# fchchen/omni-recall-rag

Measured on AMD Instinct MI355X. Metric: queries/sec at top-k=10 over N x 3072-d chunks; score delta vs C# reference in `parity`, higher is better.
Workload: dtype i8 screen + f32*f32->f64 exact re-score; 1 GPU; C3: 10000000 chunks x 3072-d fp32 on one GPU, batch=256 queries per step, top-k=10, full hybrid (cosine+keyword+recency), candidate_limit=corpus; corpus_rows=10000000

## Files before the change

### omni-recall-rag_amd/csrc/orr_api.hip

```cpp
#include <hip/hip_runtime.h>

#include <algorithm>
#include <cmath>
#include <cstdarg>
#include <cstdio>
#include <chrono>
#include <pthread.h>
#include <dlfcn.h>
#include <atomic>
#include <condition_variable>
#include <functional>
#include <cstring>
#include <limits>
#include <mutex>
#include <shared_mutex>
#include <deque>
#include <new>
#include <numeric>
#include <string>
#include <string_view>
#include <thread>
#include <unordered_map>
#include <vector>

#include "orr_escalation.h"
#include "orr_insert_plan.h"
#include "orr_kernels.h"
#include "orr_keyword_plan.h"
#include "orr_lanes.h"
#include "orr_scope_plan.h"
#include "orr_mask_plan.h"
#include "orr_group_plan.h"
#include "orr_scope_set_plan.h"
#include "orr_scope_terms_plan.h"
#include "orr_scope_near_plan.h"
#include "orr_range_bulk_plan.h"
#include "orr_cluster_handle_plan.h"
#include "orr_cluster_group_plan.h"
#include "orr_cluster_scope_plan.h"
#include "orr_cluster_diverse_plan.h"
#include "orr_cluster_per_key_plan.h"
#include "orr_token_index.h"

namespace {

thread_local std::string g_last_error = "";

int fail(int code, const char *fmt, ...)
{
    char buf[512];
    va_list ap;
    va_start(ap, fmt);
    vsnprintf(buf, sizeof(buf), fmt, ap);
    va_end(ap);
    g_last_error = buf;
    return code;
}

// ... 2630 lines not shown
    Empty,
    Exact,
    StreamMfma,
    SplitAll,
    SplitFused,
    TwoStageGemm,
    TwoStageStream,
    LargeK,
};

enum class Screen { None, I8Ranges, GemvI8, GemvBf16, Bf16Shadow, Bf16x1 };

struct PassPlan {
    PassForm form = PassForm::Exact;
    Screen screen = Screen::None;
    bool use_cos = false;
    bool use_mfma = false;
    bool q_on_device = false;
    bool dev_norms = false;
    bool prefix_i8 = false;
    bool split_queries = false;
    bool batched_score = false;
    bool rowc_inline = false;
    int32_t fused_sample_seg = 0;
    int64_t dotf_rows = 0;
    int n_ranges = 1;
    int64_t range_row[17] = {};
    int32_t count_bits = 0;
    int prefix_floor_form = 0;
    double approx_eps = 0.0;
    double eps1 = 0.0;
    bool masked = false;
    bool grouped = false;

    bool two_stage() const {
        return form == PassForm::TwoStageGemm || form == PassForm::TwoStageStream;
    }
    bool stream() const { return form == PassForm::TwoStageStream; }
    double plane_bytes_per_row(int32_t B) const { return (count_bits == 2 ? 8.0 : 16.0) * (double)((B + 31) / 32); }
    bool fused() const { return fused_sample_seg > 0; }
    int pass_mode() const { static constexpr int kMode[] = {0, 1, 1, 2, 2, 3}; return grouped ? 6 : masked ? 5 : kMode[(int)screen]; }
};

static bool has_tiny_query(const float *q, int32_t B, int32_t D)
{
    for (int32_t b = 0; b < B; ++b) {
        float mx = 0.f;
        for (int32_t k = 0; k < D; ++k) mx = std::max(mx, std::fabs(q[(size_t)b * D + k]));
        if (mx > 0.f && mx < 0x1p-48f) return true;
    }
    return false;
}

int plan_form(orr_index *idx, const BatchArgs &a, int32_t kprime, int64_t n, const std::vector<uint32_t> &qoff, PassPlan &p)
{
    const int32_t B = a.B, D = idx->dim;
    const int32_t n_seg_all = (int32_t)((n + orr::kSelSegRows - 1) / orr::kSelSegRows);
    const bool small_k = kprime <= orr::kSelWidth;
    const bool floor_fits = !a.no_fuse && n_seg_all >= 48 && std::max<int32_t>(1, a.topk) <= orr::kSelWidth;
    p = PassPlan{};
    p.use_cos = a.dim > 0 && a.dim == D;
    p.q_on_device = p.use_cos && is_device_pointer(a.q);
    const bool force_exact = a.force_exact || (p.use_cos && (idx->opt_two_stage != 1 || D % 128 != 0) && !p.q_on_device &&
                                               has_tiny_query(a.q, B, D));
    bool stream = false, stream_i8 = false;
    if (p.use_cos && !force_exact && idx->opt_two_stage == 1 && D % 64 == 0 && small_k && floor_fits && B <= orr::kMaxGemvScreenQ) {
// ... 90 lines not shown
    const uint32_t *chunks = nullptr;
    int64_t words = 0;
    std::vector<int64_t> took, n_clip, sample;
    const int64_t *d_clip = nullptr;
    const int64_t *d_sample = nullptr;
    bool floor_heads = false;
    std::vector<int32_t> qgroup;
    uint32_t cap = 0;
    const uint32_t *d_qgroup = nullptr;
    const int64_t *d_took = nullptr;
    uint32_t *h_screened = nullptr;
};

struct PassIo {
    const float *d_q = nullptr;
    double *d_dot = nullptr;
    float *d_dotf = nullptr;
    orr::KwView kw{nullptr, 0, nullptr, nullptr, nullptr};
    const double2 *d_rowc = nullptr;
    orr_candidate *d_cand = nullptr;
    bool direct_host = false;
    const MaskScope *mask = nullptr;
    GroupScopes *groups = nullptr;
};

struct PassFront {
    std::vector<uint32_t> qoff;
    uint32_t n_terms_total = 0;
    size_t rec_bytes = 0;
    bool q_download_pending = false;
    PassIo io;
};

template <class Plan>
int open_pass(orr_index *idx, const BatchArgs &a, int32_t kprime, Plan &&plan, bool pinned_records, bool out_dev, bool dev_norms,
              const float **q_host, PassPlan &p, PassFront &f)
{
    const int32_t B = a.B;
    hipStream_t s = idx->stream;
    if (q_host) *q_host = nullptr;
    f.qoff.resize((size_t)B + 1);
    memcpy(f.qoff.data(), a.query_term_off, sizeof(uint32_t) * ((size_t)B + 1));
    for (int32_t b = 0; b < B; ++b) {
        if (f.qoff[b + 1] < f.qoff[b]) return fail(ORR_EINVAL, "query_term_off is not monotone at query %d", b);
        if (f.qoff[b + 1] - f.qoff[b] > 65535) return fail(ORR_EINVAL, "query %d has more than 65535 terms", b);
    }
    f.n_terms_total = f.qoff[B] - f.qoff[0];
    if (f.n_terms_total > 0 && (!a.term_off || !a.terms_utf8)) return fail(ORR_EINVAL, "terms are referenced but term_off/terms_utf8 is NULL");

    ORR_TRY(plan(f.qoff, p));
    if (!dev_norms) p.dev_norms = false;
    idx->h_survivors.clear();

    PassIo &io = f.io;
    f.rec_bytes = sizeof(orr_candidate) * (size_t)B * ((size_t)kprime + 1);
    io.direct_host = pinned_records && !p.use_mfma && f.rec_bytes <= (256u << 10);
    if (io.direct_host) {
        ORR_TRY(idx->pin_cand.reserve(f.rec_bytes));
        io.d_cand = idx->pin_cand.as<orr_candidate>();
    } else if (out_dev && a.out_dev) {
        io.d_cand = a.out_dev;
    } else {
        ORR_TRY(idx->ws_cand.reserve(f.rec_bytes));
        io.d_cand = idx->ws_cand.as<orr_candidate>();
    }

    idx->h_norm_a.assign((size_t)B, 0.0);
    if (!p.use_cos) return ORR_OK;
    const size_t qbytes = sizeof(float) * (size_t)B * a.dim;
    if (p.dev_norms) {
        io.d_q = a.q;
        ORR_TRY(idx->ws_norm_a.reserve(sizeof(double) * (size_t)B));
        ORR_TRY(idx->pin_norm.reserve(sizeof(double) * (size_t)B));
        HIP_TRY(orr::launch_dot_exact(io.d_q, B, a.dim, nullptr, 1, true, idx->ws_norm_a.as<double>(), B, idx->stream_aux));
        HIP_TRY(hipEventRecord(idx->ev_q, idx->stream_aux));
        return ORR_OK;
    }
    ORR_TRY(idx->pin_q.reserve(qbytes));
    if (p.q_on_device) {
        io.d_q = a.q;
        HIP_TRY(hipMemcpyAsync(idx->pin_q.p, a.q, qbytes, hipMemcpyDeviceToHost, idx->stream_kw));
        HIP_TRY(hipEventRecord(idx->ev_q, idx->stream_kw));
        f.q_download_pending = true;
    } else {
// ... 173 lines not shown
        if (host_records && !a.out_dev && rec_bytes <= (256u << 10)) {
            ORR_TRY(idx->pin_cand.reserve(rec_bytes));
            io.d_cand = idx->pin_cand.as<orr_candidate>();
            io.direct_host = true;
        }
        Timed t(idx, "finish_survivors", 0.0);
        HIP_TRY(orr::launch_finish_survivors(idx->d_emb, idx->dim, io.d_q, B, idx->d_norm_b, idx->d_created, idx->d_row_ids, io.kw,
                                             idx->ws_qc.as<orr::QueryConst>(), a.now_ticks, epi.cnt, idx->ws_fcnt.as<uint32_t>() + 2 * B,
                                             kCap, epi.buf, idx->ws_fdot.as<double>(), idx->ws_sel.as<orr::SelEntry>(), kprime, n,
                                             idx->row_base, idx->ws_tsL.as<double>(), io.d_cand, idx->pin_cnt.as<uint32_t>(), s));
    } else {
        ORR_TRY(rescore_survivors(idx, a, io, epi, kCap, how, rescore_bytes, s));
        {
            Timed t(idx, "buffer_to_lists", 0.0);
            HIP_TRY(orr::launch_buffer_to_lists(epi.buf, epi.cnt, kCap, B, 0, buf_lists, idx->ws_sel.as<orr::SelEntry>(), s));
        }
        {
            Timed t(idx, "select_final", (double)B * (double)buf_lists * orr::kSelWidth * sizeof(orr::SelEntry));
            HIP_TRY(orr::launch_select_final(idx->ws_sel.as<orr::SelEntry>(), buf_lists, B, kprime, n, idx->row_base,
                                             nullptr, nullptr, 0, idx->d_norm_b, idx->d_created, idx->d_row_ids, io.kw,
                                             0, 0.0, nullptr, epi.cnt, kCap, idx->ws_tsL.as<double>(), io.d_cand, s));
        }
        {
            Timed t(idx, "records_dot_from_buffer", 0.0);
            HIP_TRY(orr::launch_records_dot_from_buffer(epi.buf, idx->ws_fdot.as<double>(), epi.cnt, kCap, B, kprime, idx->row_base,
                                                        io.d_cand, s));
        }
        if (how == Rescore::BufferExact)
            HIP_TRY(hipMemcpyAsync(idx->pin_cnt.p, epi.cnt, sizeof(uint32_t) * (size_t)B, hipMemcpyDeviceToHost, s));
    }
    return ORR_OK;
}

int screen_i8_in_ranges(orr_index *idx, const BatchArgs &a, const PassPlan &p, int64_t n, const orr::KwView &kw,
                        orr::FusedEpilogue epi, hipStream_t s)
{
    const int32_t B = a.B;
    const int64_t *range_row = p.range_row;
    if (p.n_ranges > 1) {
        hipStream_t k = idx->stream_kw;
        HIP_TRY(hipEventRecord(idx->ev_main_ready, s));
        HIP_TRY(hipStreamWaitEvent(k, idx->ev_main_ready, 0));
        for (int r = 1; r < p.n_ranges; ++r) {
            {
                Timed t(idx, "count_planes", p.plane_bytes_per_row(B) * (double)(range_row[r + 1] - range_row[r]), k);
                HIP_TRY(orr::launch_query_count_planes(kw, B, n, epi.plane_stride, idx->ws_fany.as<uint32_t>(), k, range_row[r],
                                                       range_row[r + 1], epi.count_bits == 2 ? 2 : 4));
            }
            HIP_TRY(hipEventRecord(idx->ev_range[r - 1], k));
        }
    }
    for (int r = 0; r < p.n_ranges; ++r) {
        if (r > 0) HIP_TRY(hipStreamWaitEvent(s, idx->ev_range[r - 1], 0));
        epi.tickets = idx->ws_tickets.as<uint32_t>() + 8 * r;
        const double rows_r = (double)(range_row[r + 1] - range_row[r]);
        Timed t(idx, "screen_i8_fused", rows_r * ((double)idx->dim + 32.0 + (epi.count_planes ? (epi.count_bits == 2 ? 8.0 : 16.0) * (double)((B + 31) / 32) : 0.0)) +
                                        1.0 * (double)B * idx->dim);
        HIP_TRY(orr::launch_screen_i8(idx->ws_qtiled.p, B, idx->emb_i8.p, range_row[r + 1], idx->dim, epi, s, range_row[r]));
    }
    return ORR_OK;
}

orr_index *capture_handle(orr_index *lane) { return lane->internal_lane && lane->parent ? const_cast<orr_index *>(lane->parent) : lane; }

int capture_screen(orr_index *idx, const BatchArgs &a, const PassPlan &p, int64_t n, const PassIo &io, const orr::FloorOut &floor,
                   const orr::FusedEpilogue &epi, uint32_t kCap, int32_t kth, hipStream_t s)
{
    ScreenCapture &c = capture_handle(idx)->capture;
    const size_t B = (size_t)a.B;
    c.armed.store(0, std::memory_order_relaxed);
    c.have = false;
    c.floor_key.resize(B); c.L.resize(B); c.cnt.resize(B); c.buf.resize(B * (size_t)kCap);
    HIP_TRY(hipMemcpyAsync(c.floor_key.data(), floor.floor_key, sizeof(unsigned long long) * B, hipMemcpyDeviceToHost, s));
    HIP_TRY(hipMemcpyAsync(c.L.data(), floor.L, sizeof(double) * B, hipMemcpyDeviceToHost, s));
    HIP_TRY(hipMemcpyAsync(c.cnt.data(), epi.cnt, sizeof(uint32_t) * B, hipMemcpyDeviceToHost, s));
    HIP_TRY(hipMemcpyAsync(c.buf.data(), epi.buf, sizeof(orr::SelEntry) * B * (size_t)kCap, hipMemcpyDeviceToHost, s));
    HIP_TRY(hipStreamSynchronize(s));
    orr_screen_capture &o = c.info;
    o = orr_screen_capture{};
    o.B = a.B; o.kth = kth; o.cap = kCap;
    o.screen = (int32_t)p.screen;
    o.tile_form = p.screen == Screen::I8Ranges ? orr::screen_i8_form(a.B, p.range_row[1], idx->dim, epi) : -1;
    o.scope = io.groups ? 2 : io.mask ? 1 : 0;
    o.floor_form = io.mask || p.stream() ? -1 : p.prefix_floor_form;
    o.n = n;
    o.prefix_rows = io.mask ? io.mask->sample : std::min<int64_t>(p.dotf_rows, n);
// ... 88 lines not shown
                HIP_TRY(orr::launch_screen_gemv_i8(idx->ws_q8.p, idx->ws_q8s1.as<float>(), idx->ws_q8err.as<double>(), B, idx->emb_i8.p,
                                                   idx->i8_scale.as<float>(), idx->i8_rel_err.as<float>(), idx->i8_rel_hat.as<float>(),
                                                   idx->d_norm_b, idx->d_created, a.now_ticks, pre_rows, idx->dim, pre, true, s));
            else
                HIP_TRY(orr::launch_screen_gemv_bf16(idx->ws_qsplit.p, B, idx->emb_shadow.p, pre_rows, idx->dim, pre, s));
        }
        {
            Timed t(idx, "select_floor", 0.0);
            const int32_t lists_all = (int32_t)(cap_p / orr::kSelWidth);
            const int32_t lists_p = pre_lists ? (int32_t)((pre_rows + orr::kSelWidth - 1) / orr::kSelWidth) : lists_all;
            if (!pre_lists)
                HIP_TRY(orr::launch_buffer_to_lists(pre.buf, pre.cnt, cap_p, B, 0, lists_all, idx->ws_psel.as<orr::SelEntry>(), s));
            HIP_TRY(orr::launch_select_final_sample(idx->ws_psel.as<orr::SelEntry>(), lists_all, lists_p, B, kth, d_tau, s, floor));
        }
    } else {
        if (!io.mask) {
            Timed t(idx, "select_floor", 0.0);
            HIP_TRY(orr::launch_select_final_sample(idx->ws_sel.as<orr::SelEntry>(), lists_total, p.fused_sample_seg, B, kth, d_tau, s, floor,
                                                    p.prefix_floor_form == 2 ? 1 : 0));
        }
        const bool gemm_i8 = p.screen == Screen::I8Ranges;
        if (gemm_i8) {
            epi.i8_rowf = idx->i8_rowf.as<float4>();
            epi.i8_qs1 = idx->ws_q8s1.as<float>();
        }
        HIP_TRY(orr::launch_fused_query_consts(idx->ws_qc.as<orr::QueryConst>(), idx->ws_tskey.as<unsigned long long>(), B,
                                               idx->ws_fqf.as<float4>(), s, gemm_i8 ? idx->ws_q8s1.as<float>() : nullptr,
                                               gemm_i8 ? idx->ws_q8err.as<double>() + B : nullptr,
                                               gemm_i8 ? idx->ws_fqf.as<float4>() + B : nullptr,
                                               idx->ws_fcnt.as<uint32_t>(), 3 * B, idx->ws_tickets.as<uint32_t>(), 8 * 16));
        epi.qf16 = gemm_i8 ? idx->ws_fqf.as<float4>() + B : nullptr;
    }
    epi.tau = idx->ws_tskey.as<unsigned long long>();
    if (p.screen == Screen::I8Ranges) {
        ORR_TRY(screen_i8_in_ranges(idx, a, p, n, io.kw, epi, s));
    } else if (p.screen == Screen::GemvI8) {
        Timed t(idx, "screen_gemv_i8", 1.0 * (double)n * idx->dim + 28.0 * (double)n + 2.0 * (double)B * idx->dim);
        HIP_TRY(orr::launch_screen_gemv_i8(idx->ws_q8.p, idx->ws_q8s1.as<float>(), idx->ws_q8err.as<double>(), B, idx->emb_i8.p,
                                           idx->i8_scale.as<float>(), idx->i8_rel_err.as<float>(), idx->i8_rel_hat.as<float>(),
                                           io.mask ? nullptr : idx->d_norm_b, idx->d_created, a.now_ticks, n, idx->dim, epi, false, s));
    } else if (p.screen == Screen::GemvBf16) {
        Timed t(idx, "screen_gemv_bf16", 2.0 * (double)n * idx->dim + 2.0 * (double)B * idx->dim);
        HIP_TRY(orr::launch_screen_gemv_bf16(idx->ws_qsplit.p, B, idx->emb_shadow.p, n, idx->dim, epi, s));
    } else if (p.screen == Screen::Bf16Shadow) {
        ORR_TRY(idx->ws_qtiled.reserve(orr::bf16_tiled_bytes(B, idx->dim)));
        HIP_TRY(orr::launch_bf16_tiled(io.d_q, B, idx->dim, idx->ws_qtiled.p, s));
        Timed t(idx, "screen_bf16_fused", 2.0 * (double)n * idx->dim + 2.0 * (double)B * idx->dim);
        HIP_TRY(orr::launch_screen_bf16(idx->ws_qtiled.p, B, idx->emb_shadow.p, 0, n, idx->dim, nullptr, 0, &epi, s));
    } else {
        Timed t(idx, "gemm_dot_bf16x1_fused", 4.0 * (double)n * idx->dim + 2.0 * (double)B * idx->dim);
        HIP_TRY(orr::launch_gemm_dot_bf16x3(idx->ws_qsplit.p, B, idx->d_emb, 0, n, idx->dim, nullptr, 0, &epi, 1, s));
    }
    if (io.groups) {
        if (idx->profiling == 1 && io.groups->h_screened)
            HIP_TRY(hipMemcpyAsync(io.groups->h_screened, epi.cnt, sizeof(uint32_t) * (size_t)B, hipMemcpyDeviceToHost, s));
        Timed t(idx, "mask_survivors_grouped", 16.0 * (double)B * (double)kCap);
        HIP_TRY(orr::launch_mask_survivors_grouped(io.groups->bm, io.groups->words, io.groups->n_groups, io.groups->d_clip, io.groups->d_qgroup,
                                                   epi.cnt, kCap, epi.buf, B, s));
    } else if (io.mask) {
        Timed t(idx, "mask_survivors", 16.0 * (double)B * (double)kCap);
        HIP_TRY(orr::launch_mask_survivors(io.mask->bm, io.mask->n_clip, epi.cnt, kCap, epi.buf, B, s));
    }
    if (capture_handle(idx)->capture.armed.load(std::memory_order_relaxed)) ORR_TRY(capture_screen(idx, a, p, n, io, floor, epi, kCap, kth, s));
    ORR_TRY(two_stage_tail(idx, a, kprime, n, io, epi, kCap, buf_lists, host_records, rec_bytes, Rescore::BufferExact, 0.0, s));
    if (io.groups) HIP_TRY(orr::launch_mask_trailers_grouped(io.d_cand, B, kprime, io.groups->d_took, s));
    else if (io.mask) HIP_TRY(orr::launch_mask_trailers(io.d_cand, B, kprime, io.mask->took, s));
// ... 2 lines not shown

int select_fused(orr_index *idx, const BatchArgs &a, const PassPlan &p, int32_t kprime, int64_t n, PassIo &io, bool host_records,
                 size_t rec_bytes)
{
    const int32_t B = a.B;
    hipStream_t s = idx->stream;
    uint32_t kCap = idx->survivor_cap;
    if (io.groups && io.groups->cap) kCap = io.groups->cap;
    while (kCap > 8192 && (size_t)B * kCap * 40 > ((size_t)2 << 30)) kCap >>= 1;
    idx->pass_cap = kCap;
    const int32_t fss = p.fused_sample_seg;
    const int32_t buf_lists = (int32_t)(kCap / orr::kSelWidth);
    const int32_t lists_total = fss + buf_lists;
    const int32_t finish_group = orr::finish_survivors_group(B, idx->dim);
    const int32_t lists_room = std::max<int32_t>(lists_total, finish_group ? (int32_t)(kCap / (uint32_t)finish_group) : 0);
    ORR_TRY(idx->ws_sel.reserve(sizeof(orr::SelEntry) * (size_t)B * (size_t)lists_room * orr::kSelWidth));
    ORR_TRY(idx->ws_tau.reserve(sizeof(unsigned long long) * (size_t)B));
    ORR_TRY(idx->ws_fcnt.reserve(sizeof(uint32_t) * 3 * (size_t)B));
    ORR_TRY(idx->ws_fbuf.reserve(sizeof(orr::SelEntry) * (size_t)B * kCap));
    unsigned long long *d_tau = idx->ws_tau.as<unsigned long long>();
    if (!p.stream() && !io.mask) {
        Timed t(idx, "fuse_select", (double)B * (double)p.dotf_rows * 28.0);
        orr::I8Prefix i8p;
        if (p.prefix_i8) { i8p.rowf = idx->i8_rowf.as<float4>(); i8p.qs1 = idx->ws_q8s1.as<float>(); i8p.qerr2 = idx->ws_q8err.as<double>() + B; }
        HIP_TRY(orr::launch_fuse_select(nullptr, io.d_dotf, p.dotf_rows, idx->d_norm_b, idx->d_created, io.d_rowc, io.kw,
                                        idx->ws_qc.as<orr::QueryConst>(), a.now_ticks, std::min<int64_t>(p.dotf_rows, n), B, 0, fss,
                                        nullptr, idx->ws_sel.as<orr::SelEntry>(), lists_total, s, i8p,
                                        p.prefix_floor_form));
    }
    ORR_TRY(idx->ws_fqf.reserve(sizeof(float4) * 2 * (size_t)B));
    orr::FusedEpilogue epi{};
    epi.plane_stride = (n + 63) / 64 * 64;
    if (io.kw.bitmaps && !p.stream()) {
        ORR_TRY(idx->ws_fany.reserve(sizeof(uint32_t) * orr::kCountPlanes * (size_t)((B + 31) / 32) * (size_t)epi.plane_stride));
        epi.count_bits = p.count_bits;
        Timed t(idx, "count_planes", p.plane_bytes_per_row(B) * (double)(p.range_row[1] - p.range_row[0]));
        HIP_TRY(orr::launch_query_count_planes(io.kw, B, n, epi.plane_stride, idx->ws_fany.as<uint32_t>(), s, 0, p.range_row[1],
                                               epi.count_bits == 2 ? 2 : 4));
        epi.count_planes = idx->ws_fany.as<uint32_t>();
    }
    epi.qf = idx->ws_fqf.as<float4>();
    epi.rowc = io.d_rowc; epi.qc = idx->ws_qc.as<orr::QueryConst>(); epi.kw = io.kw;
    epi.cnt = idx->ws_fcnt.as<uint32_t>(); epi.buf = idx->ws_fbuf.as<orr::SelEntry>(); epi.cap = kCap;
    if (p.screen == Screen::GemvBf16) HIP_TRY(hipMemsetAsync(idx->ws_fcnt.p, 0, sizeof(uint32_t) * 3 * (size_t)B, s));
    ORR_TRY(idx->ws_tickets.reserve(sizeof(uint32_t) * 8 * 16));
    if (p.two_stage()) return screen_two_stage(idx, a, p, kprime, n, io, epi, kCap, buf_lists, lists_total, host_records, rec_bytes);

    {
        Timed t(idx, "select_floor", 0.0);
        HIP_TRY(orr::launch_select_final_sample(idx->ws_sel.as<orr::SelEntry>(), lists_total, fss, B, kprime, d_tau, s));
    }
    HIP_TRY(orr::launch_fused_query_consts(idx->ws_qc.as<orr::QueryConst>(), d_tau, B, idx->ws_fqf.as<float4>(), s, nullptr, nullptr, nullptr,
                                           idx->ws_fcnt.as<uint32_t>(), 3 * B));
    epi.tau = d_tau;
    {
        Timed t(idx, "gemm_dot_bf16x3_fused", 4.0 * (double)(n - p.dotf_rows) * idx->dim + 4.0 * (double)B * idx->dim);
        HIP_TRY(orr::launch_gemm_dot_bf16x3(idx->ws_qsplit.p, B, idx->d_emb, p.dotf_rows, n, idx->dim, nullptr, 0, &epi, 3, s));
    }
    {
        Timed t(idx, "buffer_to_lists", 0.0);
        HIP_TRY(orr::launch_buffer_to_lists(epi.buf, epi.cnt, kCap, B, fss, lists_total, idx->ws_sel.as<orr::SelEntry>(), s));
    }
    Timed t(idx, "select_final", (double)B * (double)lists_total * orr::kSelWidth * sizeof(orr::SelEntry));
    HIP_TRY(orr::launch_select_final(idx->ws_sel.as<orr::SelEntry>(), lists_total, B, kprime, n, idx->row_base,
                                     nullptr, nullptr, 0, idx->d_norm_b, idx->d_created, idx->d_row_ids, io.kw,
                                     0, p.approx_eps, nullptr, epi.cnt, kCap, nullptr, io.d_cand, s));
    return ORR_OK;
}

int launch_selection(orr_index *idx, const BatchArgs &a, const PassPlan &p, int32_t kprime, int64_t n, PassIo &io, bool host_records,
                     size_t rec_bytes)
{
    const int32_t B = a.B;
    hipStream_t s = idx->stream;
    if (p.form == PassForm::LargeK)
        return run_large_k(idx, a, kprime, n, io.d_dot, io.kw, idx->pin_qc.as<orr::QueryConst>(), io.d_cand, s);
    const int64_t n_seg = (n + orr::kSelSegRows - 1) / orr::kSelSegRows;
    const int32_t n_seg32 = (int32_t)n_seg;
    ORR_TRY(idx->ws_sel.reserve(sizeof(orr::SelEntry) * (size_t)B * (size_t)n_seg * orr::kSelWidth));
    if (p.fused()) {
        ORR_TRY(select_fused(idx, a, p, kprime, n, io, host_records, rec_bytes));
    } else {
        const orr::QueryConst *qc = idx->ws_qc.as<orr::QueryConst>();
        unsigned long long *d_tau = nullptr;
        const int32_t sample_seg = (B >= 8 && n_seg32 >= 48) ? std::min<int32_t>(64, std::max<int32_t>(16, n_seg32 / 16)) : 0;
        if (sample_seg > 0) {
            ORR_TRY(idx->ws_tau.reserve(sizeof(unsigned long long) * (size_t)B));
// ... 80 lines not shown
    }
    g_ht.mark(4);
    collect_events(idx);
    return check_hit_list(idx, kws, nullptr);
}

int run_shard_once(orr_index *idx, const BatchArgs &a, int32_t kprime, bool host_records, const float **q_host,
                   const orr_candidate **recs_host, PassPlan &p)
{
    g_ht.start();
    ORR_TRY(bind_device(idx));
    const int64_t n = participating_rows(idx, a.candidate_limit);
    const int32_t B = a.B;
    hipStream_t s = idx->stream;
    if (recs_host) *recs_host = nullptr;

    PassFront f;
    ORR_TRY(open_pass(idx, a, kprime, [&](const std::vector<uint32_t> &qoff, PassPlan &plan) { return plan_pass(idx, a, kprime, n, qoff, plan); },
                      host_records, true, true, q_host, p, f));
    PassIo &io = f.io;

    if (p.form == PassForm::Empty) {
        const std::vector<orr_candidate> empty = empty_records(B, kprime);
        if (io.direct_host) memcpy(io.d_cand, empty.data(), f.rec_bytes);
        else HIP_TRY(hipMemcpyAsync(io.d_cand, empty.data(), f.rec_bytes, hipMemcpyHostToDevice, s));
        HIP_TRY(hipStreamSynchronize(s));
        if (f.q_download_pending || p.dev_norms) HIP_TRY(hipEventSynchronize(idx->ev_q));
        if (recs_host && io.direct_host) *recs_host = io.d_cand;
        return ORR_OK;
    }

    if (p.screen == Screen::GemvI8) ORR_TRY(launch_i8_query_image(idx, io.d_q, B, false, s));

    KwSide kws;
    ORR_TRY(launch_keyword_side(idx, a, f.qoff, kws));
    io.kw = kws.view;
    g_ht.mark(1);

    ORR_TRY(launch_numerators(idx, a, p, n, io));
    g_ht.mark(0);

    ORR_TRY(launch_consts(idx, a, p, n, f.qoff, f.q_download_pending, io));
    if (f.n_terms_total > 0) HIP_TRY(hipStreamWaitEvent(s, idx->ev_kw_done, 0));
    g_ht.mark(2);

    ORR_TRY(launch_selection(idx, a, p, kprime, n, io, host_records, f.rec_bytes));

    if (!owner_of(idx)->dead.empty())
        HIP_TRY(orr::launch_mark_dead_records(io.d_cand, B, kprime, owner_of(idx)->d_dead.as<int64_t>(),
                                              (int32_t)owner_of(idx)->dead.size(), idx->row_base, s));
    if (host_records) ORR_TRY(records_to_host(idx, f, s));
    g_ht.mark(3);
    idx->sstats.pass_mode = p.pass_mode();

    const int r = finish_pass(idx, a, p, kws, f.n_terms_total);
    if (r != ORR_OK) return r;
    if (recs_host && io.direct_host) *recs_host = io.d_cand;
    else if (recs_host && host_records) *recs_host = idx->pin_cand.as<orr_candidate>();
    return ORR_OK;
}

template <class Pass>
int retry_pass(orr_index *idx, Pass &&once)
{
    for (int attempt = 0;; ++attempt) {
        const int r = once();
        if (r != kRetryPass) return r;
        idx->sstats.passes += 1;
        if (attempt + 1 >= keyword::kMaxRuns) return hit_list_kept_overflowing(nullptr);
    }
}

int run_shard(orr_index *idx, const BatchArgs &a, int32_t kprime, bool host_records, const float **q_host,
              const orr_candidate **recs_host, PassPlan &pass)
{
    return retry_pass(idx, [&] { return run_shard_once(idx, a, kprime, host_records, q_host, recs_host, pass); });
// ... 616 lines not shown
}


struct ScopeSource {
    const ScopeArgs *list = nullptr;
    const orr_scope *handle = nullptr;
    bool empty() const { return handle ? handle->live.load() <= 0 : list->n_ids == 0; }
};

constexpr int kNotMaskable = 2;

int run_masked_pass(orr_index *idx, const BatchArgs &a, int32_t kprime, const MaskScope &ms, const float **q_host,
                    const orr_candidate **recs_host, PassPlan &p, GroupScopes *groups = nullptr)
{
    ORR_TRY(bind_device(idx));
    const int64_t n = ms.n_clip;
    const int32_t B = a.B;
    hipStream_t s = idx->stream;
    *recs_host = nullptr;
    PassFront f;
    auto plan = [&](const std::vector<uint32_t> &qoff, PassPlan &pl) -> int {
        ORR_TRY(plan_pass(idx, a, kprime, n, qoff, pl));
        if (!pl.two_stage()) return kNotMaskable;
        pl.masked = true;
        pl.grouped = groups != nullptr;
        pl.rowc_inline = false;
        return ORR_OK;
    };
    ORR_TRY(open_pass(idx, a, kprime, plan, true, false, false, q_host, p, f));
    PassIo &io = f.io;
    io.mask = &ms;
    io.groups = groups;
    if (p.screen == Screen::GemvI8) ORR_TRY(launch_i8_query_image(idx, io.d_q, B, false, s));
    KwSide kws;
    ORR_TRY(launch_keyword_side(idx, a, f.qoff, kws));
    io.kw = kws.view;
    ORR_TRY(launch_numerators(idx, a, p, n, io));
    ORR_TRY(launch_consts(idx, a, p, n, f.qoff, f.q_download_pending, io));
    if (f.n_terms_total > 0) HIP_TRY(hipStreamWaitEvent(s, idx->ev_kw_done, 0));
    ORR_TRY(launch_selection(idx, a, p, kprime, n, io, true, f.rec_bytes));
    ORR_TRY(records_to_host(idx, f, s));
    idx->sstats.pass_mode = p.pass_mode();
    const int r = finish_pass(idx, a, p, kws, f.n_terms_total);
    if (r != ORR_OK) return r;
    if (groups && groups->h_screened && idx->profiling == 1) {
        double pairs = 0.0;
        for (int32_t b = 0; b < B; ++b) pairs += (double)std::min<uint32_t>(groups->h_screened[b], idx->pass_cap);
        add_phase_stat(idx, "grouped_screen_pairs", std::chrono::steady_clock::now(), 16.0 * pairs);
    }
    *recs_host = io.direct_host ? io.d_cand : idx->pin_cand.as<orr_candidate>();
    return ORR_OK;
}

int list_part_records(orr_index *idx, const BatchArgs &orig, const ScopeSlice &call_sl, const MaskScope &ms, const std::vector<int32_t> &gids,
                      scope::Form form, int64_t K, bool requery, std::vector<orr_candidate> &store, std::vector<double> &norms)
{
    ScopeSlice sl = call_sl;
    const bool all = form == scope::Form::AllRecords;
    const int64_t part_rows = idx->opt_mask_part_rows;
    const int64_t P = mask::part_count(ms.took, part_rows);
    hipStream_t s = idx->stream;
    uint32_t *h_live = const_cast<uint32_t *>(sl.live), *h_took = const_cast<uint32_t *>(sl.took);
    const size_t nb = gids.size(), rec_q = (size_t)K + 1;
    const std::vector<uint32_t> q(gids.begin(), gids.end());
    store.assign((size_t)P * nb * rec_q, orr_candidate{});
    norms.assign(nb, 0.0);
    if (P > 1) {
        ORR_TRY(idx->ws_scope_bm.reserve(sizeof(uint32_t) * (size_t)sl.words));
        ORR_TRY(idx->ws_scope_chunks.reserve(sizeof(uint32_t) * (size_t)orr::scope_chunks(sl.words)));
        sl.bm = idx->ws_scope_bm.as<uint32_t>(); sl.chunks = idx->ws_scope_chunks.as<uint32_t>();
    }
    for (int64_t j = 0; j < P; ++j) {
// ... 5086 lines not shown
```

Measured before the change: 31670 queries/s.

## Plan front-stage stream/event ordering; launch vector side before keyword chain for GEMM

```diff
diff --git a/omni-recall-rag_amd/csrc/host/orr_front_plan_selftest.cpp b/omni-recall-rag_amd/csrc/host/orr_front_plan_selftest.cpp
--- /dev/null
+++ b/omni-recall-rag_amd/csrc/host/orr_front_plan_selftest.cpp
@@ -0,0 +1,248 @@
+#include "../orr_front_plan.h"
+
+#include <cstdio>
+#include <string>
+#include <vector>
+
+using namespace front;
+
+static long g_fail = 0;
+static std::string g_case;
+#define CHECK(c)                                                                                                                  \
+    do {                                                                                                                          \
+        if (!(c)) { ++g_fail; if (g_fail < 40) fprintf(stderr, "FAIL %s:%d: %s   [%s]\n", __FILE__, __LINE__, #c, g_case.c_str()); } \
+    } while (0)
+
+enum Res { Vectors, Norms, Images, Dots, Bitmaps, Qc, Rowc, Lists, FloorKeys, Fqf, Words0, Buf0 = Words0 + kMaxRanges, kRes = Buf0 + kMaxRanges };
+
+struct Io { std::vector<int> reads, writes; };
+
+static Io io_of(const Facts &f, const Step &s)
+{
+    const bool gemm = f.form == Form::TwoStageGemm, strm = f.form == Form::TwoStageStream;
+    const bool fused = gemm || strm || f.form == Form::SplitFused;
+    const bool words = f.has_terms && fused && !strm;
+    const bool masked = f.masked && (gemm || strm);
+    Io io;
+    switch (s.stage) {
+    case Stage::Queries:
+        if (!f.q_on_device) io.writes = {Vectors};
+        else io.writes = {Norms};
+        break;
+    case Stage::QueryImages: io.reads = {Vectors}; io.writes = {Images}; break;
+    case Stage::Prefix: io.reads = {Vectors, Images}; io.writes = {Dots}; break;
+    case Stage::KeywordChain: io.writes = {Bitmaps}; break;
+    case Stage::NormsPatch: io.reads = {Norms}; io.writes = {Qc}; break;
+    case Stage::RowConsts: io.writes = {Rowc}; break;
+    case Stage::PrefixSelect: io.reads = {Dots, Qc, Rowc, Bitmaps}; io.writes = {Lists}; break;
+    case Stage::CountWords: io.reads = {Bitmaps}; io.writes = {Words0 + s.range}; break;
+    case Stage::Floor:
+        if (masked) io.reads = {Vectors, Qc, Bitmaps};
+        else if (strm) io.reads = {Images, Qc, Rowc, Bitmaps};
+        else io.reads = {Lists};
+        io.writes = {FloorKeys};
+        break;
+    case Stage::QueryConsts: io.reads = {Qc, FloorKeys}; io.writes = {Fqf}; break;
+    case Stage::Gemm:
+        io.reads = {Images, Rowc, Qc, FloorKeys, Bitmaps};
+        if (!strm) io.reads.push_back(Fqf);
+        if (words) io.reads.push_back(Words0 + s.range);
+        io.writes = {Buf0 + s.range};
+        break;
+    case Stage::Tail:
+        io.reads = {Vectors, Qc, Bitmaps};
+        break;
+    }
+    return io;
+}
+
+static bool made(const Facts &f, const Plan &p, int res)
+{
+    for (int i = 0; i < p.n; ++i)
+        for (int w : io_of(f, p.steps[i]).writes)
+            if (w == res) return true;
+    return false;
+}
+
+static bool ordered(const Plan &p, int w, int c)
+{
+    if (w >= c) return false;
+    const Step &W = p.steps[w], &C = p.steps[c];
+    if (W.stream == C.stream) return true;
+    for (int r = w; r < c; ++r) {
+        const Step &R = p.steps[r];
+        if (R.stream != W.stream || R.record == kEvNone) continue;
+        for (int x = r + 1; x <= c; ++x) {
+            const Step &X = p.steps[x];
+            const bool waits = X.wait[0] == R.record || X.wait[1] == R.record;
+            if (waits && (X.stream == C.stream || X.host_waits)) return true;
+        }
+    }
+    for (int m = w + 1; m < c; ++m)
+        if (p.steps[m].stream != W.stream && p.steps[m].stream != C.stream && ordered(p, w, m) && ordered(p, m, c)) return true;
+    return false;
+}
+
+static const char *stage_name(Stage s)
+{
+    static const char *n[] = {"Queries", "QueryImages", "Prefix", "KeywordChain", "NormsPatch", "RowConsts", "PrefixSelect", "CountWords", "Floor",
+                              "QueryConsts", "Gemm", "Tail"};
+    return n[(int)s];
+}
+
+static std::string sequence(const Plan &p)
+{
+    std::string out;
+    for (int i = 0; i < p.n; ++i) {
+        const Step &s = p.steps[i];
+        if (i) out += " ";
+        out += stage_name(s.stage);
+        if (s.stage == Stage::CountWords || s.stage == Stage::Gemm) out += std::to_string((int)s.range);
+        out += s.stream == Stream::Main ? "" : s.stream == Stream::Keyword ? "@kw" : "@aux";
+    }
+    return out;
+}
+
+static void check_plan(const Facts &f, long &steps_checked, long &edges_checked)
+{
+    const Plan p = front_plan(f);
+    CHECK(p.n >= 2 && p.n <= Plan::kMaxSteps);
+    CHECK(p.steps[0].stage == Stage::Queries && p.steps[p.n - 1].stage == Stage::Tail && p.steps[p.n - 1].stream == Stream::Main);
+    for (int i = 0; i < p.n; ++i)
+        for (int j = i + 1; j < p.n; ++j) CHECK(!(p.steps[i].stage == p.steps[j].stage && p.steps[i].range == p.steps[j].range));
+    for (int c = 0; c < p.n; ++c) {
+        for (int res : io_of(f, p.steps[c]).reads) {
+            if (!made(f, p, res)) continue;
+            bool found = false, all = true;
+            for (int w = 0; w < p.n; ++w) {
+                bool writes = false;
+                for (int x : io_of(f, p.steps[w]).writes) writes |= x == res;
+                if (!writes) continue;
+                found = true;
+                if (!ordered(p, w, c)) {
+                    all = false;
+                    if (g_fail < 40) fprintf(stderr, "  %s%d reads what %s%d writes, unordered\n", stage_name(p.steps[c].stage), p.steps[c].range, stage_name(p.steps[w].stage), p.steps[w].range);
+                }
+                ++edges_checked;
+            }
+            CHECK(found && all);
+        }
+        ++steps_checked;
+    }
+    int recorded_at[kEvents];
+    for (int &r : recorded_at) r = -1;
+    for (int i = 0; i < p.n; ++i) {
+        const Step &s = p.steps[i];
+        for (int8_t w : s.wait)
+            if (w != kEvNone) CHECK(w >= 0 && w < kEvents && recorded_at[w] >= 0 && recorded_at[w] < i);
+        if (s.host_waits) CHECK(s.wait[0] != kEvNone);
+        if (s.record != kEvNone) {
+            CHECK(s.record >= 0 && s.record < kEvents && recorded_at[s.record] < 0);
+            if (s.record >= 0 && s.record < kEvents) recorded_at[s.record] = i;
+        }
+    }
+    for (int e = 0; e < kEvents; ++e) {
+        if (recorded_at[e] < 0) continue;
+        bool joined = false;
+        for (int i = recorded_at[e] + 1; i < p.n && !joined; ++i) {
+            const Step &s = p.steps[i];
+            if (s.wait[0] != e && s.wait[1] != e) continue;
+            if (s.stream == Stream::Main || s.host_waits) joined = true;
+            else
+                for (int m = i; m < p.n && !joined; ++m)
+                    if (p.steps[m].stream == s.stream && p.steps[m].record != kEvNone)
+                        for (int x = m + 1; x < p.n; ++x)
+                            if (p.steps[x].stream == Stream::Main && (p.steps[x].wait[0] == p.steps[m].record || p.steps[x].wait[1] == p.steps[m].record)) joined = true;
+        }
+        CHECK(joined);
+    }
+    for (int i = 0; i < p.n; ++i) {
+        const Step &s = p.steps[i];
+        if (s.stage == Stage::CountWords && s.stream == Stream::Keyword) CHECK(s.range >= 1 && p.index(Stage::QueryConsts) >= 0 && p.index(Stage::QueryConsts) < i);
+        if (s.stage == Stage::CountWords)
+            CHECK(p.words_site(s.range) == (s.stream == Stream::Main ? Plan::Words::InSelection : Plan::Words::BesideGemm));
+    }
+    CHECK(p.words_site(kMaxRanges) == Plan::Words::None);
+    for (int i = 0; i < p.n; ++i) CHECK(p.steps[i].record != kEvWords && p.steps[i].wait[0] != kEvWords && p.steps[i].wait[1] != kEvWords);
+}
+
+static std::string legacy_sequence(const Facts &f)
+{
+    const bool download = f.q_on_device && !f.dev_norms;
+    std::string q = std::string("Queries") + (f.dev_norms ? "@aux" : download ? "@kw" : "");
+    if (f.form == Form::Empty) return q + " Tail";
+    const std::string kw = f.has_terms ? " KeywordChain@kw" : "";
+    switch (f.form) {
+    case Form::Exact: case Form::LargeK: case Form::StreamMfma:
+        return q + kw + " Prefix NormsPatch RowConsts PrefixSelect Tail";
+    case Form::SplitAll:
+        return q + kw + " QueryImages Prefix NormsPatch RowConsts PrefixSelect Tail";
+    case Form::SplitFused:
+        return q + kw + " QueryImages Prefix NormsPatch RowConsts PrefixSelect" + (f.has_terms ? " CountWords0" : "") + " Floor QueryConsts Gemm0 Tail";
+    case Form::TwoStageStream:
+        if (f.screen == Screen::GemvI8) return q + " QueryImages" + kw + " NormsPatch RowConsts Floor Gemm0 Tail";
+        return q + kw + " QueryImages NormsPatch RowConsts Floor Gemm0 Tail";
+    default: return "";
+    }
+}
+
+int main()
+{
+    long plans = 0, steps = 0, edges = 0, legacy = 0, gemm_plans = 0;
+    const int ranges[] = {1, 2, 3, 4, 8, 16};
+    for (int form = 0; form <= (int)Form::LargeK; ++form)
+        for (int screen = 0; screen <= (int)Screen::Bf16x1; ++screen)
+            for (int nr : ranges)
+                for (int bits = 0; bits < 32; ++bits) {
+                    Facts f;
+                    f.form = (Form)form; f.screen = (Screen)screen; f.n_ranges = nr;
+                    f.has_terms = bits & 1; f.masked = bits & 2; f.grouped = bits & 4; f.dev_norms = bits & 8; f.q_on_device = bits & 16;
+                    if (f.grouped && !f.masked) continue;
+                    if (f.dev_norms && !f.q_on_device) continue;
+                    g_case = "form " + std::to_string(form) + " screen " + std::to_string(screen) + " ranges " + std::to_string(nr) + " bits " + std::to_string(bits);
+                    const Plan p = front_plan(f);
+                    g_case += ": " + sequence(p);
+                    check_plan(f, steps, edges);
+                    ++plans;
+                    if (f.form != Form::TwoStageGemm) {
+                        CHECK(sequence(p) == legacy_sequence(f));
+                        for (int i = 0; i < p.n; ++i)
+                            CHECK(p.steps[i].stage == Stage::Queries || p.steps[i].stage == Stage::KeywordChain || p.steps[i].stream == Stream::Main);
+                        ++legacy;
+                        continue;
+                    }
+                    ++gemm_plans;
+                    CHECK(p.index(Stage::QueryImages) == 1);
+                    CHECK(f.masked ? !p.has(Stage::Prefix) && !p.has(Stage::PrefixSelect) : p.index(Stage::Prefix) == 2);
+                    if (f.has_terms) {
+                        CHECK(p.before(Stage::QueryImages, Stage::KeywordChain) && p.before(Stage::KeywordChain, Stage::NormsPatch));
+                        const int n_launch = f.screen == Screen::I8Ranges ? nr : 1;
+                        for (int r = 0; r < n_launch; ++r) {
+                            CHECK(p.has(Stage::CountWords, r) && p.has(Stage::Gemm, r));
+                            if (!p.has(Stage::CountWords, r) || !p.has(Stage::Gemm, r)) continue;
+                            const Step &w = p.at(Stage::CountWords, r), &g = p.at(Stage::Gemm, r);
+                            CHECK(w.stream == (r > 0 ? Stream::Keyword : Stream::Main));
+                            if (r == 0) CHECK(w.record == kEvNone && g.wait[0] == kEvNone && p.index(Stage::PrefixSelect) < p.index(Stage::CountWords, 0));
+                            if (r > 0) CHECK(w.record == kEvWords + r && g.wait[0] == kEvWords + r && (w.wait[0] == kEvMainReady) == (r == 1));
+                            if (r > 0) CHECK(p.index(Stage::QueryConsts) < p.index(Stage::CountWords, r) && p.at(Stage::QueryConsts).record == kEvMainReady);
+                        }
+                        CHECK(!p.has(Stage::CountWords, n_launch) && !p.has(Stage::Gemm, n_launch));
+                    } else {
+                        for (int i = 0; i < p.n; ++i) CHECK(p.steps[i].stage != Stage::CountWords && p.steps[i].stage != Stage::KeywordChain);
+                    }
+                }
+    {
+        Facts f;
+        f.form = Form::TwoStageGemm; f.screen = Screen::I8Ranges; f.n_ranges = 4; f.has_terms = true; f.dev_norms = true; f.q_on_device = true;
+        g_case = "headline";
+        const std::string want = "Queries@aux QueryImages Prefix KeywordChain@kw NormsPatch RowConsts PrefixSelect CountWords0 Floor QueryConsts "
+                                 "CountWords1@kw CountWords2@kw CountWords3@kw Gemm0 Gemm1 Gemm2 Gemm3 Tail";
+        CHECK(sequence(front_plan(f)) == want);
+        printf("headline: %s\n", sequence(front_plan(f)).c_str());
+    }
+    printf("plans checked: %ld (GEMM two-stage: %ld, in the order they always had: %ld)\n", plans, gemm_plans, legacy);
+    printf("steps checked: %ld, producer edges checked: %ld\n", steps, edges);
+    if (g_fail) { printf("orr_front_plan_selftest: %ld FAILED\n", g_fail); return 1; }
+    printf("orr_front_plan_selftest: ok\n");
+    return 0;
+}
diff --git a/omni-recall-rag_amd/csrc/orr_api.hip b/omni-recall-rag_amd/csrc/orr_api.hip
--- a/omni-recall-rag_amd/csrc/orr_api.hip
+++ b/omni-recall-rag_amd/csrc/orr_api.hip
@@ -24,6 +24,7 @@
 #include <vector>
 
 #include "orr_escalation.h"
+#include "orr_front_plan.h"
 #include "orr_insert_plan.h"
 #include "orr_kernels.h"
 #include "orr_keyword_plan.h"
@@ -2720,6 +2721,7 @@
     double eps1 = 0.0;
     bool masked = false;
     bool grouped = false;
+    front::Plan front;
 
     bool two_stage() const {
         return form == PassForm::TwoStageGemm || form == PassForm::TwoStageStream;
@@ -2876,6 +2878,53 @@
     PassIo io;
 };
 
+static_assert((int)PassForm::Empty == (int)front::Form::Empty && (int)PassForm::Exact == (int)front::Form::Exact &&
+              (int)PassForm::StreamMfma == (int)front::Form::StreamMfma && (int)PassForm::SplitAll == (int)front::Form::SplitAll &&
+              (int)PassForm::SplitFused == (int)front::Form::SplitFused && (int)PassForm::TwoStageGemm == (int)front::Form::TwoStageGemm &&
+              (int)PassForm::TwoStageStream == (int)front::Form::TwoStageStream && (int)PassForm::LargeK == (int)front::Form::LargeK, "front::Form");
+static_assert((int)Screen::None == (int)front::Screen::None && (int)Screen::I8Ranges == (int)front::Screen::I8Ranges &&
+              (int)Screen::GemvI8 == (int)front::Screen::GemvI8 && (int)Screen::GemvBf16 == (int)front::Screen::GemvBf16 &&
+              (int)Screen::Bf16Shadow == (int)front::Screen::Bf16Shadow && (int)Screen::Bf16x1 == (int)front::Screen::Bf16x1, "front::Screen");
+static_assert(front::kMaxRanges == 16, "ev_range: one event per row range but the first");
+
+front::Facts front_facts(const PassPlan &p, bool has_terms)
+{
+    front::Facts f;
+    f.form = (front::Form)(int)p.form;
+    f.screen = (front::Screen)(int)p.screen;
+    f.n_ranges = p.n_ranges;
+    f.has_terms = has_terms;
+    f.masked = p.masked; f.grouped = p.grouped;
+    f.dev_norms = p.dev_norms; f.q_on_device = p.q_on_device;
+    return f;
+}
+
+hipStream_t front_stream(const orr_index *idx, front::Stream on)
+{
+    return on == front::Stream::Main ? idx->stream : on == front::Stream::Keyword ? idx->stream_kw : idx->stream_aux;
+}
+
+hipEvent_t front_event(const orr_index *idx, int8_t ev)
+{
+    if (ev == front::kEvQ) return idx->ev_q;
+    if (ev == front::kEvKwDone) return idx->ev_kw_done;
+    if (ev == front::kEvMainReady) return idx->ev_main_ready;
+    assert(ev > front::kEvWords && ev < front::kEvents);
+    return idx->ev_range[ev - front::kEvWords - 1];
+}
+
+int front_waits(const orr_index *idx, const front::Step &st)
+{
+    for (int8_t ev : st.wait)
+        if (ev != front::kEvNone) HIP_TRY(hipStreamWaitEvent(front_stream(idx, st.stream), front_event(idx, ev), 0));
+    return ORR_OK;
+}
+int front_record(const orr_index *idx, const front::Step &st)
+{
+    if (st.record != front::kEvNone) HIP_TRY(hipEventRecord(front_event(idx, st.record), front_stream(idx, st.stream)));
+    return ORR_OK;
+}
+
 template <class Plan>
 int open_pass(orr_index *idx, const BatchArgs &a, int32_t kprime, Plan &&plan, bool pinned_records, bool out_dev, bool dev_norms,
               const float **q_host, PassPlan &p, PassFront &f)
@@ -2894,6 +2943,7 @@
 
     ORR_TRY(plan(f.qoff, p));
     if (!dev_norms) p.dev_norms = false;
+    p.front = front::front_plan(front_facts(p, f.n_terms_total > 0));
     idx->h_survivors.clear();
 
     PassIo &io = f.io;
@@ -3133,26 +3183,33 @@
     return ORR_OK;
 }
 
+int reserve_count_words(orr_index *idx, int32_t B, int64_t n)
+{
+    return idx->ws_fany.reserve(sizeof(uint32_t) * orr::kCountPlanes * (size_t)((B + 31) / 32) * (size_t)((n + 63) / 64 * 64));
+}
+int launch_count_words(orr_index *idx, const BatchArgs &a, const PassPlan &p, int64_t n, const orr::KwView &kw, int r)
+{
+    const front::Step &st = p.front.at(front::Stage::CountWords, r);
+    hipStream_t k = front_stream(idx, st.stream);
+    ORR_TRY(front_waits(idx, st));
+    {
+        Timed t(idx, "count_planes", p.plane_bytes_per_row(a.B) * (double)(p.range_row[r + 1] - p.range_row[r]), k);
+        HIP_TRY(orr::launch_query_count_planes(kw, a.B, n, (n + 63) / 64 * 64, idx->ws_fany.as<uint32_t>(), k, p.range_row[r], p.range_row[r + 1],
+                                               p.count_bits == 2 ? 2 : 4));
+    }
+    return front_record(idx, st);
+}
+
 int screen_i8_in_ranges(orr_index *idx, const BatchArgs &a, const PassPlan &p, int64_t n, const orr::KwView &kw,
                         orr::FusedEpilogue epi, hipStream_t s)
 {
     const int32_t B = a.B;
     const int64_t *range_row = p.range_row;
-    if (p.n_ranges > 1) {
-        hipStream_t k = idx->stream_kw;
-        HIP_TRY(hipEventRecord(idx->ev_main_ready, s));
-        HIP_TRY(hipStreamWaitEvent(k, idx->ev_main_ready, 0));
-        for (int r = 1; r < p.n_ranges; ++r) {
-            {
-                Timed t(idx, "count_planes", p.plane_bytes_per_row(B) * (double)(range_row[r + 1] - range_row[r]), k);
-                HIP_TRY(orr::launch_query_count_planes(kw, B, n, epi.plane_stride, idx->ws_fany.as<uint32_t>(), k, range_row[r],
-                                                       range_row[r + 1], epi.count_bits == 2 ? 2 : 4));
-            }
-            HIP_TRY(hipEventRecord(idx->ev_range[r - 1], k));
-        }
-    }
+    ORR_TRY(front_record(idx, p.front.at(front::Stage::QueryConsts)));
+    for (int r = 0; r < p.n_ranges; ++r)
+        if (p.front.words_site(r) == front::Plan::Words::BesideGemm) ORR_TRY(launch_count_words(idx, a, p, n, kw, r));
     for (int r = 0; r < p.n_ranges; ++r) {
-        if (r > 0) HIP_TRY(hipStreamWaitEvent(s, idx->ev_range[r - 1], 0));
+        ORR_TRY(front_waits(idx, p.front.at(front::Stage::Gemm, r)));
         epi.tickets = idx->ws_tickets.as<uint32_t>() + 8 * r;
         const double rows_r = (double)(range_row[r + 1] - range_row[r]);
         Timed t(idx, "screen_i8_fused", rows_r * ((double)idx->dim + 32.0 + (epi.count_planes ? (epi.count_bits == 2 ? 8.0 : 16.0) * (double)((B + 31) / 32) : 0.0)) +
@@ -3307,6 +3364,7 @@
         epi.qf16 = gemm_i8 ? idx->ws_fqf.as<float4>() + B : nullptr;
     }
     epi.tau = idx->ws_tskey.as<unsigned long long>();
+    if (p.screen != Screen::I8Ranges) ORR_TRY(front_waits(idx, p.front.at(front::Stage::Gemm)));
     if (p.screen == Screen::I8Ranges) {
         ORR_TRY(screen_i8_in_ranges(idx, a, p, n, io.kw, epi, s));
     } else if (p.screen == Screen::GemvI8) {
@@ -3375,11 +3433,10 @@
     orr::FusedEpilogue epi{};
     epi.plane_stride = (n + 63) / 64 * 64;
     if (io.kw.bitmaps && !p.stream()) {
-        ORR_TRY(idx->ws_fany.reserve(sizeof(uint32_t) * orr::kCountPlanes * (size_t)((B + 31) / 32) * (size_t)epi.plane_stride));
+        ORR_TRY(reserve_count_words(idx, B, n));
         epi.count_bits = p.count_bits;
-        Timed t(idx, "count_planes", p.plane_bytes_per_row(B) * (double)(p.range_row[1] - p.range_row[0]));
-        HIP_TRY(orr::launch_query_count_planes(io.kw, B, n, epi.plane_stride, idx->ws_fany.as<uint32_t>(), s, 0, p.range_row[1],
-                                               epi.count_bits == 2 ? 2 : 4));
+        assert(p.front.words_site(0) == front::Plan::Words::InSelection);
+        ORR_TRY(launch_count_words(idx, a, p, n, io.kw, 0));
         epi.count_planes = idx->ws_fany.as<uint32_t>();
     }
     epi.qf = idx->ws_fqf.as<float4>();
@@ -3396,6 +3453,7 @@
     HIP_TRY(orr::launch_fused_query_consts(idx->ws_qc.as<orr::QueryConst>(), d_tau, B, idx->ws_fqf.as<float4>(), s, nullptr, nullptr, nullptr,
                                            idx->ws_fcnt.as<uint32_t>(), 3 * B));
     epi.tau = d_tau;
+    ORR_TRY(front_waits(idx, p.front.at(front::Stage::Gemm)));
     {
         Timed t(idx, "gemm_dot_bf16x3_fused", 4.0 * (double)(n - p.dotf_rows) * idx->dim + 4.0 * (double)B * idx->dim);
         HIP_TRY(orr::launch_gemm_dot_bf16x3(idx->ws_qsplit.p, B, idx->d_emb, p.dotf_rows, n, idx->dim, nullptr, 0, &epi, 3, s));
@@ -3542,16 +3600,18 @@
 
     if (p.screen == Screen::GemvI8) ORR_TRY(launch_i8_query_image(idx, io.d_q, B, false, s));
 
+    const bool vector_first = p.front.before(front::Stage::QueryImages, front::Stage::KeywordChain);
+    if (vector_first) ORR_TRY(launch_numerators(idx, a, p, n, io));
+    g_ht.mark(0);
     KwSide kws;
     ORR_TRY(launch_keyword_side(idx, a, f.qoff, kws));
     io.kw = kws.view;
     g_ht.mark(1);
-
-    ORR_TRY(launch_numerators(idx, a, p, n, io));
+    if (!vector_first) ORR_TRY(launch_numerators(idx, a, p, n, io));
     g_ht.mark(0);
 
     ORR_TRY(launch_consts(idx, a, p, n, f.qoff, f.q_download_pending, io));
-    if (f.n_terms_total > 0) HIP_TRY(hipStreamWaitEvent(s, idx->ev_kw_done, 0));
+    if (p.front.has(front::Stage::KeywordChain)) HIP_TRY(hipStreamWaitEvent(s, idx->ev_kw_done, 0));
     g_ht.mark(2);
 
     ORR_TRY(launch_selection(idx, a, p, kprime, n, io, host_records, f.rec_bytes));
@@ -4234,12 +4294,14 @@
     io.mask = &ms;
     io.groups = groups;
     if (p.screen == Screen::GemvI8) ORR_TRY(launch_i8_query_image(idx, io.d_q, B, false, s));
+    const bool vector_first = p.front.before(front::Stage::QueryImages, front::Stage::KeywordChain);
+    if (vector_first) ORR_TRY(launch_numerators(idx, a, p, n, io));
     KwSide kws;
     ORR_TRY(launch_keyword_side(idx, a, f.qoff, kws));
     io.kw = kws.view;
-    ORR_TRY(launch_numerators(idx, a, p, n, io));
+    if (!vector_first) ORR_TRY(launch_numerators(idx, a, p, n, io));
     ORR_TRY(launch_consts(idx, a, p, n, f.qoff, f.q_download_pending, io));
-    if (f.n_terms_total > 0) HIP_TRY(hipStreamWaitEvent(s, idx->ev_kw_done, 0));
+    if (p.front.has(front::Stage::KeywordChain)) HIP_TRY(hipStreamWaitEvent(s, idx->ev_kw_done, 0));
     ORR_TRY(launch_selection(idx, a, p, kprime, n, io, true, f.rec_bytes));
     ORR_TRY(records_to_host(idx, f, s));
     idx->sstats.pass_mode = p.pass_mode();
diff --git a/omni-recall-rag_amd/csrc/orr_front_plan.h b/omni-recall-rag_amd/csrc/orr_front_plan.h
--- /dev/null
+++ b/omni-recall-rag_amd/csrc/orr_front_plan.h
@@ -0,0 +1,130 @@
+#pragma once
+
+#include <cstdint>
+
+namespace front {
+
+enum class Form : int8_t { Empty, Exact, StreamMfma, SplitAll, SplitFused, TwoStageGemm, TwoStageStream, LargeK };
+enum class Screen : int8_t { None, I8Ranges, GemvI8, GemvBf16, Bf16Shadow, Bf16x1 };
+
+struct Facts {
+    Form form = Form::Exact;
+    Screen screen = Screen::None;
+    int n_ranges = 1;
+    bool has_terms = false;
+    bool masked = false, grouped = false;
+    bool dev_norms = false;
+    bool q_on_device = false;
+};
+
+enum class Stream : int8_t { Main, Keyword, Aux };
+
+enum class Stage : int8_t {
+    Queries,
+    QueryImages,
+    Prefix,
+    KeywordChain,
+    NormsPatch,
+    RowConsts,
+    PrefixSelect,
+    CountWords,
+    Floor,
+    QueryConsts,
+    Gemm,
+    Tail,
+};
+
+constexpr int kMaxRanges = 16;
+
+constexpr int8_t kEvNone = -1, kEvQ = 0, kEvKwDone = 1, kEvMainReady = 2, kEvWords = 3;
+constexpr int kEvents = kEvWords + kMaxRanges;
+
+struct Step {
+    Stage stage = Stage::Tail;
+    int8_t range = 0;
+    Stream stream = Stream::Main;
+    int8_t record = kEvNone;
+    int8_t wait[2] = {kEvNone, kEvNone};
+    bool host_waits = false;
+};
+
+struct Plan {
+    static constexpr int kMaxSteps = 12 + 2 * kMaxRanges;
+    Step steps[kMaxSteps];
+    int n = 0;
+
+    int index(Stage st, int range = 0) const
+    {
+        for (int i = 0; i < n; ++i)
+            if (steps[i].stage == st && steps[i].range == range) return i;
+        return -1;
+    }
+    bool has(Stage st, int range = 0) const { return index(st, range) >= 0; }
+    const Step &at(Stage st, int range = 0) const { return steps[index(st, range)]; }
+    bool before(Stage first, Stage second) const { return has(first) && has(second) && index(first) < index(second); }
+    enum class Words { None, InSelection, BesideGemm };
+    Words words_site(int r) const
+    {
+        const int w = index(Stage::CountWords, r);
+        if (w < 0) return Words::None;
+        return w < index(Stage::QueryConsts) ? Words::InSelection : Words::BesideGemm;
+    }
+};
+
+inline Plan front_plan(const Facts &f)
+{
+    Plan p;
+    auto add = [&](Stage st, Stream on, int8_t record = kEvNone, int8_t wait0 = kEvNone, int8_t wait1 = kEvNone, int range = 0) -> Step & {
+        Step &s = p.steps[p.n++];
+        s.stage = st; s.range = (int8_t)range; s.stream = on; s.record = record; s.wait[0] = wait0; s.wait[1] = wait1;
+        return s;
+    };
+    const bool download = f.q_on_device && !f.dev_norms;
+    add(Stage::Queries, f.dev_norms ? Stream::Aux : download ? Stream::Keyword : Stream::Main, f.dev_norms || download ? kEvQ : kEvNone);
+    if (f.form == Form::Empty) {
+        Step &t = add(Stage::Tail, Stream::Main, kEvNone, f.dev_norms || download ? kEvQ : kEvNone);
+        t.host_waits = f.dev_norms || download;
+        return p;
+    }
+    const bool gemm = f.form == Form::TwoStageGemm;
+    const bool stream_form = f.form == Form::TwoStageStream;
+    const bool fused = gemm || stream_form || f.form == Form::SplitFused;
+    const int n_launch = !(gemm && f.screen == Screen::I8Ranges) || f.n_ranges < 1 ? 1 : f.n_ranges > kMaxRanges ? kMaxRanges : f.n_ranges;
+    const bool words = f.has_terms && fused && !stream_form;
+    const bool prefix = !stream_form && !(gemm && f.masked);
+    const bool images = gemm || stream_form || f.form == Form::SplitAll || f.form == Form::SplitFused;
+    const bool vector_first = gemm || (stream_form && f.screen == Screen::GemvI8);
+
+    auto vector_side = [&] {
+        if (images) add(Stage::QueryImages, Stream::Main);
+        if (prefix) add(Stage::Prefix, Stream::Main);
+    };
+    if (vector_first) vector_side();
+    if (f.has_terms) add(Stage::KeywordChain, Stream::Keyword, kEvKwDone);
+    if (!vector_first) vector_side();
+    {
+        Step &c = add(Stage::NormsPatch, Stream::Main, kEvNone, f.dev_norms || download ? kEvQ : kEvNone);
+        c.host_waits = download;
+    }
+    add(Stage::RowConsts, Stream::Main);
+    int8_t join = f.has_terms ? kEvKwDone : kEvNone;
+    auto joined = [&] { const int8_t j = join; join = kEvNone; return j; };
+    if (!fused) {
+        add(Stage::PrefixSelect, Stream::Main, kEvNone, joined());
+        add(Stage::Tail, Stream::Main);
+        return p;
+    }
+    if (prefix) add(Stage::PrefixSelect, Stream::Main, kEvNone, joined());
+    if (words) add(Stage::CountWords, Stream::Main, kEvNone, joined(), kEvNone, 0);
+    add(Stage::Floor, Stream::Main, kEvNone, joined());
+    const bool late_words = words && n_launch > 1;
+    if (!stream_form) add(Stage::QueryConsts, Stream::Main, late_words ? kEvMainReady : kEvNone);
+    if (late_words)
+        for (int r = 1; r < n_launch; ++r)
+            add(Stage::CountWords, Stream::Keyword, (int8_t)(kEvWords + r), r == 1 ? kEvMainReady : kEvNone, kEvNone, r);
+    for (int r = 0; r < n_launch; ++r) add(Stage::Gemm, Stream::Main, kEvNone, late_words && r >= 1 ? (int8_t)(kEvWords + r) : kEvNone, kEvNone, r);
+    add(Stage::Tail, Stream::Main);
+    return p;
+}
+
+}
```

Result: no change. 31630 queries/s (-0.1%).
